# Gaurav14cs17/Bayer_Low_light_Image_Enhancement

Measured on AMD Instinct MI355X. Metric: megapixels/sec RawFormer-S 512x512 RAW->sRGB, higher is better.
Workload: dtype f32; 1 GPU; RawFormer-S(FLCA) dim=32, batch=8 of packed 4x512x512 synthetic Bayer per GPU; frames_per_gpu=8, variant=flca, weights=synthetic (seeded, random-init scale), parallelism=batch-sharded x1, device=AMD Radeon Graphics

## Files before the change

### bayer_low_light_image_enhancement_amd/csrc/rf_gemm1x1.hip

```cpp
#include <cstdio>
#include <cstdlib>
#include <type_traits>
#include "rf_common.h"

namespace rf {

__device__ __forceinline__ const float* kset_base(const Conv1x1Args& a, int b, int s) {
    const int k = 4 * s;
    const bool first = k < a.C1;
    const float* src = first ? a.x1 : a.x2;
    const size_t off = (size_t)b * (size_t)(first ? a.x1_bstride : a.x2_bstride) + (size_t)(first ? k : k - a.C1) * (size_t)a.P;
    return src + off;
}

__device__ __forceinline__ float4 ldv(const float* __restrict__ base, unsigned off) {
    return *reinterpret_cast<const float4*>(base + off);
}

template <int NCO>
__device__ __forceinline__ void zero_acc(f32x4 (&acc)[NCO][4]) {
#pragma unroll
    for (int t = 0; t < NCO; ++t)
#pragma unroll
        for (int g = 0; g < 4; ++g) acc[t][g] = (f32x4){0.f, 0.f, 0.f, 0.f};
}

template <class BP>
__device__ __forceinline__ void b3_split_pair(float xa, float xb, BP& bp, int g, int hp) {
    unsigned a0, a1, a2, b0, b1, b2;
    b3_split(xa, a0, a1, a2);
    b3_split(xb, b0, b1, b2);
    bp[g][0][hp] = b3_pack(a0, b0);
    bp[g][1][hp] = b3_pack(a1, b1);
    bp[g][2][hp] = b3_pack(a2, b2);
}

template <int NCO, bool RES>
__device__ __forceinline__ void epilogue(const Conv1x1Args& a, f32x4 (&acc)[NCO][4], int tfirst, int ntiles,
                                         const float* __restrict__ bias_l, const float4* res,
                                         int b, int p0, int kq, bool live) {
    const int P = a.P;
    float* outb = a.out + (size_t)b * a.out_bstride;
    if (a.mode == 0) {
        const unsigned voff = (unsigned)(4 * kq) * (unsigned)P + (unsigned)p0;
#pragma unroll
        for (int t = 0; t < NCO; ++t) {
            if (t >= ntiles) break;
#pragma unroll
            for (int r = 0; r < 4; ++r) {
                const int cu = 16 * (tfirst + t) + r;
                const float bs = bias_l[16 * t + 4 * kq + r];
                float v[4] = {acc[t][0][r] + bs, acc[t][1][r] + bs, acc[t][2][r] + bs, acc[t][3][r] + bs};
                if constexpr (RES) {
                    const float4 rv = res[t * 4 + r];
                    v[0] += rv.x; v[1] += rv.y; v[2] += rv.z; v[3] += rv.w;
                }
                if (a.act == 1 || a.act == 3) {
                    const float slope = a.act == 1 ? 0.2f : 0.1f;
#pragma unroll
                    for (int g = 0; g < 4; ++g) v[g] = v[g] > 0.f ? v[g] : slope * v[g];
                } else if (a.act == 2) {
#pragma unroll
                    for (int g = 0; g < 4; ++g) v[g] = fmaxf(v[g], 0.f);
                } else if (a.act == 4) {
#pragma unroll
                    for (int g = 0; g < 4; ++g) v[g] = fminf(fmaxf(v[g], 0.f), 1e4f);
                }
                if (live && cu + 4 * kq < a.Cout)
                    *reinterpret_cast<float4*>(outb + (size_t)cu * P + voff) = make_float4(v[0], v[1], v[2], v[3]);
            }
        }
    } else {
        const int w = a.w, w2 = 2 * a.w;
        const int ya = p0 / w, xa = p0 - ya * w;
        const int yb = (p0 + 2) / w, xb = (p0 + 2) - yb * w;
#pragma unroll
        for (int t = 0; t < NCO; ++t) {
            if (t >= ntiles) break;
            const int co = 16 * (tfirst + t) + 4 * kq;
            const int o = co >> 2;
            const float bs = bias_l[4 * t + kq];
            float* op = outb + (size_t)o * 4 * P;
            if (live && co < a.Cout) {
#pragma unroll
                for (int i = 0; i < 2; ++i) {
                    *reinterpret_cast<float4*>(op + (size_t)(2 * ya + i) * w2 + 2 * xa) =
                        make_float4(acc[t][0][2 * i] + bs, acc[t][0][2 * i + 1] + bs, acc[t][1][2 * i] + bs, acc[t][1][2 * i + 1] + bs);
                    *reinterpret_cast<float4*>(op + (size_t)(2 * yb + i) * w2 + 2 * xb) =
                        make_float4(acc[t][2][2 * i] + bs, acc[t][2][2 * i + 1] + bs, acc[t][3][2 * i] + bs, acc[t][3][2 * i + 1] + bs);
                }
            }
        }
    }
}

__device__ __forceinline__ void stage_bias(const Conv1x1Args& a, float* bias_l, int tbeg, int tpad, int tid) {
    if (a.mode == 0) {
        for (int i = tid; i < tpad * 16; i += 256) {
            const int co = 16 * tbeg + i;
            bias_l[i] = (a.bias && co < a.Cout) ? a.bias[co] : 0.f;
        }
    } else {
        for (int i = tid; i < tpad * 4; i += 256) {
            const int o = 4 * tbeg + i;
            bias_l[i] = (a.bias && 4 * o < a.Cout) ? a.bias[o] : 0.f;
        }
    }
}

template <int KS, bool LN, int RT, bool DBUF>
__global__ void __launch_bounds__(256, (KS <= 8 ? 3 : 2)) conv1x1_res_kernel(Conv1x1Args a, int ntw, int ngroups) {
    constexpr int NCO = 2;
    constexpr bool RES = RT > 0;
    extern __shared__ __attribute__((aligned(16))) float lds[];
    const int tid = threadIdx.x;
    const int lane = tid & 63, wave = tid >> 6;
    const int j = lane & 15, kq = lane >> 4;
    const int grp = blockIdx.x % ngroups;
    const int wg = blockIdx.x / ngroups, nwg = gridDim.x / ngroups;
    const int b = blockIdx.y;
    const int P = a.P;
    const int K = a.C1 + a.C2;
    const int NS = K >> 2;
    const int NT = (a.Cout + 15) >> 4;
    const int tbeg = grp * ntw;
    const int tcnt = (NT - tbeg < ntw) ? NT - tbeg : ntw;
    const int tpad = (tcnt + NCO - 1) / NCO * NCO;
    const int ntiles = (P + 255) >> 8;
    float* lds_w = lds;
    float* bias_l = lds + KS * tpad * 64;
    float* gam_l = bias_l + tpad * 16;
    float* bet_l = gam_l + 4 * KS;

    auto load_tile = [&](int tile, float4 (&dst)[KS]) {
        const int p0 = (tile * 4 + wave) * 64 + 4 * j;
        const unsigned voff = (unsigned)kq * (unsigned)P + (unsigned)(p0 < P ? p0 : 0);
#pragma unroll
        for (int s = 0; s < KS; ++s) dst[s] = ldv(kset_base(a, b, s < NS ? s : NS - 1), voff);
    };

    float4 xr[KS], xn[DBUF ? KS : 1];
    int tile = wg;
    load_tile(tile < ntiles ? tile : 0, xr);
    {
        const float* wp = a.wp + (size_t)b * a.wp_bstride;
        const int n4 = KS * tpad * 16;
        for (int idx = tid; idx < n4; idx += 256) {
            const int l4 = idx & 15;
            const int t = (idx >> 4) % tpad;
            const int s = (idx >> 4) / tpad;
            float4 v = make_float4(0.f, 0.f, 0.f, 0.f);
            if (t < tcnt && s < NS) v = *reinterpret_cast<const float4*>(wp + ((size_t)s * NT + tbeg + t) * 64 + l4 * 4);
            *reinterpret_cast<float4*>(lds_w + ((size_t)s * tpad + t) * 64 + l4 * 4) = v;
        }
        stage_bias(a, bias_l, tbeg, tpad, tid);
        if constexpr (LN) {
            for (int i = tid; i < 4 * KS; i += 256) {
                gam_l[i] = i < K ? a.ln_w[i] : 0.f;
                bet_l[i] = (a.ln_b && i < K) ? a.ln_b[i] : 0.f;
            }
        }
    }
    __syncthreads();

    for (; tile < ntiles; tile += nwg) {
        const int p0 = (tile * 4 + wave) * 64 + 4 * j;
        const bool live = p0 < P;
        const int tnext = tile + nwg;
        if constexpr (DBUF) {
            load_tile(tnext < ntiles ? tnext : tile, xn);
        }
        float4 res[RES ? RT * 4 : 1];
        if constexpr (RES) {
            const float* resb = a.res + (size_t)b * a.res_bstride;
            const unsigned voff = (unsigned)(4 * kq) * (unsigned)P + (unsigned)(live ? p0 : 0);
#pragma unroll
            for (int t = 0; t < RT; ++t)
#pragma unroll
                for (int r = 0; r < 4; ++r)
                    res[t * 4 + r] = ldv(resb + (size_t)(16 * (tbeg + (t < tcnt ? t : tcnt - 1)) + r) * P, voff);
        }
        if constexpr (LN) {
            float sum[4] = {0.f, 0.f, 0.f, 0.f};
#pragma unroll
            for (int s = 0; s < KS; ++s)
                if (s < NS) { sum[0] += xr[s].x; sum[1] += xr[s].y; sum[2] += xr[s].z; sum[3] += xr[s].w; }
            const float invK = 1.0f / (float)K;
            float mu[4], var[4] = {0.f, 0.f, 0.f, 0.f};
#pragma unroll
            for (int g = 0; g < 4; ++g) {
                sum[g] += __shfl_xor(sum[g], 16);
                sum[g] += __shfl_xor(sum[g], 32);
                mu[g] = sum[g] * invK;
            }
#pragma unroll
            for (int s = 0; s < KS; ++s) {
                if (s < NS) {
                    const float d0 = xr[s].x - mu[0], d1 = xr[s].y - mu[1], d2 = xr[s].z - mu[2], d3 = xr[s].w - mu[3];
                    var[0] = fmaf(d0, d0, var[0]); var[1] = fmaf(d1, d1, var[1]);
                    var[2] = fmaf(d2, d2, var[2]); var[3] = fmaf(d3, d3, var[3]);
                }
            }
            float rstd[4], sh[4];
#pragma unroll
            for (int g = 0; g < 4; ++g) {
                var[g] += __shfl_xor(var[g], 16);
                var[g] += __shfl_xor(var[g], 32);
                rstd[g] = 1.0f / sqrtf(var[g] * invK + a.ln_eps);
                sh[g] = a.ln_b ? mu[g] : 0.f;
            }
#pragma unroll
            for (int s = 0; s < KS; ++s) {
                const float gk = gam_l[4 * s + kq], bk = bet_l[4 * s + kq];
                xr[s].x = fmaf((xr[s].x - sh[0]) * rstd[0], gk, bk);
                xr[s].y = fmaf((xr[s].y - sh[1]) * rstd[1], gk, bk);
                xr[s].z = fmaf((xr[s].z - sh[2]) * rstd[2], gk, bk);
                xr[s].w = fmaf((xr[s].w - sh[3]) * rstd[3], gk, bk);
            }
        }
        auto do_group = [&](int tg, const float4* resp) {
            f32x4 acc[NCO][4];
            zero_acc(acc);
            const float* wl = lds_w + (size_t)tg * 64 + lane;
#pragma unroll
            for (int s = 0; s < KS; ++s) {
                const float xb[4] = {xr[s].x, xr[s].y, xr[s].z, xr[s].w};
#pragma unroll
                for (int t = 0; t < NCO; ++t) {
                    const float av = wl[((size_t)s * tpad + t) * 64];
#pragma unroll
                    for (int g = 0; g < 4; ++g)
                        acc[t][g] = __builtin_amdgcn_mfma_f32_16x16x4f32(av, xb[g], acc[t][g], 0, 0, 0);
                }
            }
            epilogue<NCO, RES>(a, acc, tbeg + tg, tcnt - tg, bias_l + (a.mode == 0 ? 16 : 4) * tg, resp, b, p0, kq, live);
        };
        if constexpr (RES) {
            do_group(0, &res[0]);
            if constexpr (RT > NCO) {
                if (tpad > NCO) do_group(NCO, &res[NCO * 4]);
            }
        } else {
#pragma unroll 1
            for (int tg = 0; tg < tpad; tg += NCO) do_group(tg, res);
        }
        if constexpr (DBUF) {
#pragma unroll
            for (int s = 0; s < KS; ++s) xr[s] = xn[s];
        } else {
            if (tnext < ntiles) load_tile(tnext, xr);
        }
    }
}

static constexpr int kStreamLnMaxK = 1024;

template <int NCO, int KCH, bool LN>
__global__ void __launch_bounds__(256, 2) conv1x1_stream_kernel(Conv1x1Args a, int ngroups) {
    __shared__ __attribute__((aligned(16))) float lds_w[2][KCH * NCO * 64];
    __shared__ float bias_l[NCO * 16];
    __shared__ float gam_l[LN ? kStreamLnMaxK : 4], bet_l[LN ? kStreamLnMaxK : 4];
    constexpr int WPT = KCH * NCO * 16 / 256;
    static_assert(KCH * NCO * 16 % 256 == 0, "weight chunk must split evenly over the workgroup");
    const int tid = threadIdx.x;
    const int lane = tid & 63, wave = tid >> 6;
    const int j = lane & 15, kq = lane >> 4;
    const int grp = blockIdx.x % ngroups;
    const int tile = blockIdx.x / ngroups;
    const int b = blockIdx.y;
    const int P = a.P;
    const int K = a.C1 + a.C2;
    const int NS = K >> 2;
    const int NT = (a.Cout + 15) >> 4;
    const int t0 = grp * NCO;
    const int tcnt = (NT - t0 < NCO) ? NT - t0 : NCO;
    const int nch = (NS + KCH - 1) / KCH;
    const int p0 = (tile * 4 + wave) * 64 + 4 * j;
    const bool live = p0 < P;
    const unsigned voff = (unsigned)kq * (unsigned)P + (unsigned)(live ? p0 : 0);
    const float* wp = a.wp + (size_t)b * a.wp_bstride;
    stage_bias(a, bias_l, t0, NCO, tid);
    if constexpr (LN) {
        for (int i = tid; i < 4 * nch * KCH; i += 256) {
            gam_l[i] = i < K ? a.ln_w[i] : 0.f;
            bet_l[i] = (a.ln_b && i < K) ? a.ln_b[i] : 0.f;
        }
    }

    f32x4 acc[NCO][4];
    zero_acc(acc);
    if (a.res && a.mode == 0) {
        const float* resb = a.res + (size_t)b * a.res_bstride;
        const unsigned vo = (unsigned)(live ? p0 : 0);
#pragma unroll
        for (int t = 0; t < NCO; ++t)
#pragma unroll
            for (int r = 0; r < 4; ++r) {
                const int co = 16 * (t0 + t) + 4 * kq + r;
                const bool ok = live && t < tcnt && co < a.Cout;
                const float4 rv = ldv(resb + (size_t)(ok ? co : 0) * P, vo);
                acc[t][0][r] = ok ? rv.x : 0.f; acc[t][1][r] = ok ? rv.y : 0.f;
                acc[t][2][r] = ok ? rv.z : 0.f; acc[t][3][r] = ok ? rv.w : 0.f;
            }
    }

    float lnA[4] = {1.f, 1.f, 1.f, 1.f}, lnB[4] = {0.f, 0.f, 0.f, 0.f};
    if constexpr (LN) {
        const float4 s4 = ldv(kset_base(a, b, 0), (unsigned)(live ? p0 : 0));
        const float sh[4] = {s4.x, s4.y, s4.z, s4.w};
        float s1[4] = {0.f, 0.f, 0.f, 0.f}, s2[4] = {0.f, 0.f, 0.f, 0.f};
#pragma unroll 16
        for (int s = 0; s < NS; ++s) {
            const float4 t = ldv(kset_base(a, b, s), voff);
            const float d[4] = {t.x - sh[0], t.y - sh[1], t.z - sh[2], t.w - sh[3]};
#pragma unroll
            for (int g = 0; g < 4; ++g) { s1[g] += d[g]; s2[g] = fmaf(d[g], d[g], s2[g]); }
        }
        const float invK = 1.0f / (float)K;
#pragma unroll
        for (int g = 0; g < 4; ++g) {
            s1[g] += __shfl_xor(s1[g], 16); s1[g] += __shfl_xor(s1[g], 32);
            s2[g] += __shfl_xor(s2[g], 16); s2[g] += __shfl_xor(s2[g], 32);
            const float md = s1[g] * invK;
            const float var = fmaxf(fmaf(-md, md, s2[g] * invK), 0.f);
            const float rstd = 1.0f / sqrtf(var + a.ln_eps);
            lnA[g] = rstd;
            lnB[g] = a.ln_b ? -(sh[g] + md) * rstd : 0.f;
        }
    }

    float4 xa[KCH], xb_[KCH], wr[WPT];
    auto load_x_chunk = [&](int c, float4 (&dst)[KCH]) {
#pragma unroll
        for (int i = 0; i < KCH; ++i) {
            const int s = c * KCH + i;
            dst[i] = ldv(kset_base(a, b, s < NS ? s : NS - 1), voff);
        }
    };
    auto load_w_chunk = [&](int c) {
#pragma unroll
        for (int i = 0; i < WPT; ++i) {
            const int idx = tid + 256 * i;
            const int l4 = idx & 15, t = (idx >> 4) % NCO, s = c * KCH + (idx >> 4) / NCO;
            const bool ok = s < NS && t < tcnt;
            const float4 v = *reinterpret_cast<const float4*>(wp + ((size_t)(ok ? s : 0) * NT + t0 + (ok ? t : 0)) * 64 + l4 * 4);
            wr[i] = ok ? v : make_float4(0.f, 0.f, 0.f, 0.f);
        }
    };
    auto store_w_chunk = [&](int buf) {
#pragma unroll
        for (int i = 0; i < WPT; ++i) *reinterpret_cast<float4*>(&lds_w[buf][(tid + 256 * i) * 4]) = wr[i];
    };
    auto chunk = [&](int c, float4 (&xc)[KCH], float4 (&xn)[KCH]) {
        if (c + 1 < nch) {
            load_x_chunk(c + 1, xn);
            load_w_chunk(c + 1);
        }
        const float* wl = &lds_w[c & 1][lane];
#pragma unroll
        for (int i = 0; i < KCH; ++i) {
            float xv[4] = {xc[i].x, xc[i].y, xc[i].z, xc[i].w};
            if constexpr (LN) {
                const int k = 4 * (c * KCH + i) + kq;
                const float gk = gam_l[k], bk = bet_l[k];
#pragma unroll
                for (int g = 0; g < 4; ++g) xv[g] = fmaf(fmaf(xv[g], lnA[g], lnB[g]), gk, bk);
            }
#pragma unroll
            for (int t = 0; t < NCO; ++t) {
                const float av = wl[(i * NCO + t) * 64];
#pragma unroll
                for (int g = 0; g < 4; ++g)
                    acc[t][g] = __builtin_amdgcn_mfma_f32_16x16x4f32(av, xv[g], acc[t][g], 0, 0, 0);
            }
        }
        if (c + 1 < nch) store_w_chunk((c + 1) & 1);
        __syncthreads();
    };

    load_x_chunk(0, xa);
    load_w_chunk(0);
    store_w_chunk(0);
    __syncthreads();
    for (int c = 0; c < nch; c += 2) {
        chunk(c, xa, xb_);
        if (c + 1 < nch) chunk(c + 1, xb_, xa);
    }
    epilogue<NCO, false>(a, acc, t0, tcnt, bias_l, nullptr, b, p0, kq, live);
}


__device__ __forceinline__ void b3_load_x_block(float4 (&xr)[8], const float* xb1, const float* xb2, const float* xb3, int C1, int C2, int C3,
                                                int c, int kq, unsigned P, unsigned pl) {
    const int cb = 32 * c;
    const bool first = cb < C1, third = cb >= C1 + C2;
    const float* src = first ? xb1 : third ? xb3 : xb2;
    const int cloc = first ? cb : third ? cb - C1 - C2 : cb - C1, cmax = (first ? C1 : third ? C3 : C2) - 1;
#pragma unroll
    for (int i = 0; i < 8; ++i) {
        int ch = cloc + 8 * kq + i;
        ch = ch < cmax ? ch : cmax;
        xr[i] = ldv(src, (unsigned)ch * P + pl);
    }
}

template <int NCO, bool LN, bool PAIR = false>
__global__ void __launch_bounds__(PAIR ? 512 : 256, 2) conv1x1_b3_kernel(Conv1x1Args a, int ngroups) {
    static_assert(!(PAIR && LN), "the paired form has no LayerNorm prologue");
    constexpr int NH = PAIR ? 2 : 1;
    __shared__ __attribute__((aligned(16))) u32x4 lds_w[NH * 2][NCO * 3 * 64];
    __shared__ float bias_l[NH * NCO * 16];
    __shared__ float gam_l[LN ? kStreamLnMaxK : 4], bet_l[LN ? kStreamLnMaxK : 4];
    constexpr int WPT = (NCO * 3 * 64 + 255) / 256;
    const int tid = PAIR ? threadIdx.x & 255 : threadIdx.x;
    const int half = PAIR ? threadIdx.x >> 8 : 0;
    const int lane = tid & 63, wave = tid >> 6;
    const int j = lane & 15, kq = lane >> 4;
    unsigned unit = 0, gp = 0, utiles = 1;
    if constexpr (PAIR) {
        utiles = (unsigned)(a.P + 255) >> 8;
        if (!conv1x1_group_map(blockIdx.x, (unsigned)a.B * utiles, (unsigned)(ngroups + 1) >> 1, &unit, &gp)) return;
    }
    const int grp = PAIR ? 2 * (int)gp + half : blockIdx.x % ngroups;
    const int tile = PAIR ? unit % utiles : blockIdx.x / ngroups;
    const int b = PAIR ? unit / utiles : blockIdx.y;
    const int P = a.P;
    const int K = a.C1 + a.C2 + a.C3;
    const int NB = (K + 31) >> 5;
    const int NT = (a.Cout + 15) >> 4;
    const bool idle = PAIR && grp >= ngroups;
    const int t0 = idle ? 0 : grp * NCO;
    const int tcnt = idle ? 0 : (NT - t0 < NCO) ? NT - t0 : NCO;
    const int p0 = (tile * 4 + wave) * 64 + 4 * j;
    const bool live = p0 < P;
    const unsigned pl = (unsigned)(live ? p0 : 0);
    const u32x4* wp3 = reinterpret_cast<const u32x4*>(reinterpret_cast<const float*>(a.wp3) + (size_t)b * a.wp3_bstride);
    stage_bias(a, bias_l + half * NCO * 16, t0, NCO, tid);
    if constexpr (LN) {
        for (int i = tid; i < 32 * NB; i += 256) {
            gam_l[i] = i < K ? a.ln_w[i] : 0.f;
            bet_l[i] = (a.ln_b && i < K) ? a.ln_b[i] : 0.f;
        }
    }

    f32x4 acc[NCO][4];
#pragma unroll
    for (int t = 0; t < NCO; ++t)
#pragma unroll
        for (int g = 0; g < 4; ++g) acc[t][g] = (f32x4){0.f, 0.f, 0.f, 0.f};
    if (a.res && a.mode == 0) {
        const float* resb = a.res + (size_t)b * a.res_bstride;
#pragma unroll
        for (int t = 0; t < NCO; ++t)
#pragma unroll
            for (int r = 0; r < 4; ++r) {
                const int co = 16 * (t0 + t) + 4 * kq + r;
                const bool ok = live && t < tcnt && co < a.Cout;
                const float4 rv = ldv(resb + (size_t)(ok ? co : 0) * P, pl);
                acc[t][0][r] = ok ? rv.x : 0.f; acc[t][1][r] = ok ? rv.y : 0.f;
                acc[t][2][r] = ok ? rv.z : 0.f; acc[t][3][r] = ok ? rv.w : 0.f;
            }
    }

    float lnA[4] = {1.f, 1.f, 1.f, 1.f}, lnB[4] = {0.f, 0.f, 0.f, 0.f};
    if constexpr (LN) {
        const unsigned voff = (unsigned)kq * (unsigned)P + pl;
        const float4 s4 = ldv(kset_base(a, b, 0), pl);
        const float sh[4] = {s4.x, s4.y, s4.z, s4.w};
        float s1[4] = {0.f, 0.f, 0.f, 0.f}, s2[4] = {0.f, 0.f, 0.f, 0.f};
#pragma unroll 16
        for (int s = 0; s < (K >> 2); ++s) {
            const float4 t = ldv(kset_base(a, b, s), voff);
            const float d[4] = {t.x - sh[0], t.y - sh[1], t.z - sh[2], t.w - sh[3]};
#pragma unroll
            for (int g = 0; g < 4; ++g) { s1[g] += d[g]; s2[g] = fmaf(d[g], d[g], s2[g]); }
        }
        const float invK = 1.0f / (float)K;
#pragma unroll
        for (int g = 0; g < 4; ++g) {
            s1[g] += __shfl_xor(s1[g], 16); s1[g] += __shfl_xor(s1[g], 32);
            s2[g] += __shfl_xor(s2[g], 16); s2[g] += __shfl_xor(s2[g], 32);
            const float md = s1[g] * invK;
            const float var = fmaxf(fmaf(-md, md, s2[g] * invK), 0.f);
            const float rstd = 1.0f / sqrtf(var + a.ln_eps);
            lnA[g] = rstd;
            lnB[g] = a.ln_b ? -(sh[g] + md) * rstd : 0.f;
        }
    }

    float4 xr[8];
    u32x4 wr[WPT];
    const float* const xb1 = a.x1 + (size_t)b * (size_t)a.x1_bstride;
    const float* const xb2 = a.x2 + (size_t)b * (size_t)a.x2_bstride;
    const float* const xb3 = a.x3 + (size_t)b * (size_t)a.x3_bstride;
    auto load_x_block = [&](int c) { b3_load_x_block(xr, xb1, xb2, xb3, a.C1, a.C2, a.C3, c, kq, (unsigned)P, pl); };
    auto load_w_block = [&](int c) {
#pragma unroll
        for (int i = 0; i < WPT; ++i) {
            const int idx = tid + 256 * i;
            const int t = idx / 192, rem = idx - t * 192;
            const bool ok = idx < NCO * 192 && t < tcnt;
            const u32x4 v = wp3[((size_t)c * NT + t0 + (ok ? t : 0)) * 192 + (ok ? rem : 0)];
            wr[i] = ok ? v : (u32x4){0u, 0u, 0u, 0u};
        }
    };
    auto store_w_block = [&](int buf) {
#pragma unroll
        for (int i = 0; i < WPT; ++i)
            if (tid + 256 * i < NCO * 192) lds_w[2 * half + buf][tid + 256 * i] = wr[i];
    };

    load_x_block(0);
    load_w_block(0);
    store_w_block(0);
    __syncthreads();
    for (int c = 0; c < NB; ++c) {
        u32x4 bp[4][3];
#pragma unroll
        for (int hp = 0; hp < 4; ++hp) {
            float xa[4] = {xr[2 * hp].x, xr[2 * hp].y, xr[2 * hp].z, xr[2 * hp].w};
            float xb[4] = {xr[2 * hp + 1].x, xr[2 * hp + 1].y, xr[2 * hp + 1].z, xr[2 * hp + 1].w};
            if constexpr (LN) {
                const int k = 32 * c + 8 * kq + 2 * hp;
                const float ga = gam_l[k], ba = bet_l[k], gb = gam_l[k + 1], bb = bet_l[k + 1];
#pragma unroll
                for (int g = 0; g < 4; ++g) {
                    xa[g] = fmaf(fmaf(xa[g], lnA[g], lnB[g]), ga, ba);
                    xb[g] = fmaf(fmaf(xb[g], lnA[g], lnB[g]), gb, bb);
                }
            }
#pragma unroll
            for (int g = 0; g < 4; ++g) b3_split_pair(xa[g], xb[g], bp, g, hp);
        }
        if (c + 1 < NB) {
            load_x_block(c + 1);
            load_w_block(c + 1);
        }
        const u32x4* wl = &lds_w[2 * half + (c & 1)][lane];
#pragma unroll
        for (int t = 0; t < NCO; ++t) {
            const u32x4 ap[3] = {wl[(t * 3 + 0) * 64], wl[(t * 3 + 1) * 64], wl[(t * 3 + 2) * 64]};
            b3_mfma4(ap, bp, acc[t]);
        }
        if (c + 1 < NB) store_w_block((c + 1) & 1);
        __syncthreads();
    }
    epilogue<NCO, false>(a, acc, t0, tcnt, bias_l + half * NCO * 16, nullptr, b, p0, kq, live);
}

template <int KB, int NCO, bool RESIDENT>
__device__ __forceinline__ void b3_ln_tiles(const Conv1x1Args& a, const int tpw, u32x4* __restrict__ Bl, float* __restrict__ red,
                                            const float* __restrict__ bias_l) {
    constexpr int KPW = KB >= 4 ? KB / 4 : 1;
    constexpr int CPT = KB >= 4 ? 8 : 4;
    constexpr int K = 32 * KB;
    constexpr int STEPS = KB * NCO, RING = RESIDENT ? STEPS : KB > 4 ? 12 : (STEPS < 5 ? STEPS : 5);
    constexpr int AHEAD = RESIDENT ? STEPS : RING - 1;
    constexpr int XSTEP = (KB == 4 && NCO == 3) ? STEPS - NCO : STEPS - RING;
    const int tid = threadIdx.x, lane = tid & 63, wave = __builtin_amdgcn_readfirstlane(tid >> 6);
    const int j = lane & 15, kq = lane >> 4;
    const int b = blockIdx.y, P = a.P;
    const int NT = a.Cout >> 4;
    const int ntile = (P + 63) >> 6;
    const int tw0 = ((int)blockIdx.z * 4 + wave) * tpw;
    const float* xb = a.x1 + (size_t)b * a.x1_bstride;
    float* outb = a.out + (size_t)b * a.out_bstride;
    const char* wp3 = reinterpret_cast<const char*>(reinterpret_cast<const float*>(a.wp3) + (size_t)b * a.wp3_bstride);
    const unsigned aoff = 16u * (unsigned)lane;

    const int kb0 = KB >= 4 ? wave * KPW : wave >> 1;
    const int cwave = KB >= 4 ? 0 : 4 * (wave & 1);
    const int cbase = 8 * kq + cwave;
    float4 xr[KPW][CPT];
    auto load_x = [&](int tile, bool exists) {
        const int q0 = tile * 64 + 4 * j;
        size_t xoff = exists ? (size_t)(8 * kq) * (size_t)P + (size_t)(q0 < P ? q0 : tile * 64) : (size_t)0;
        asm volatile("" : "+v"(xoff));
#pragma unroll
        for (int i = 0; i < KPW; ++i)
#pragma unroll
            for (int c = 0; c < CPT; ++c) xr[i][c] = *reinterpret_cast<const float4*>(xb + (size_t)(32 * (kb0 + i) + cwave + c) * (size_t)P + xoff);
    };
    u32x4 A[RING][3];
    auto load_a = [&](int slot, int step, int t0) {
        const int kb = step / NCO, t = step - kb * NCO;
#pragma unroll
        for (int pc = 0; pc < 3; ++pc)
            A[slot][pc] = *reinterpret_cast<const u32x4*>(wp3 + (((size_t)kb * NT + t0 + t) * 192 + pc * 64) * 16 + aoff);
    };
    load_x(blockIdx.x, true);
#pragma unroll
    for (int i = 0; i < AHEAD; ++i) load_a(i, i, tw0);
    constexpr bool LNREG = KB != 4;
    float gam[LNREG ? KPW : 1][CPT], bet[LNREG ? KPW : 1][CPT];
    if constexpr (LNREG) {
#pragma unroll
        for (int i = 0; i < KPW; ++i)
#pragma unroll
            for (int c = 0; c < CPT; ++c) {
                const int k = 32 * (kb0 + i) + cbase + c;
                gam[i][c] = a.ln_w[k];
                bet[i][c] = a.ln_b ? a.ln_b[k] : 0.f;
            }
    }
    __builtin_amdgcn_s_waitcnt(0x0F70);

    for (int tile = blockIdx.x; tile < ntile; tile += gridDim.x) {
    const int tnext = tile + (int)gridDim.x;
    const bool more = tnext < ntile;
    const int q0 = tile * 64 + 4 * j;
    const int p0 = q0 < P ? q0 : tile * 64;
    float mean[4], rstd[4];
    {
        float s[4] = {0.f, 0.f, 0.f, 0.f};
#pragma unroll
        for (int i = 0; i < KPW; ++i)
#pragma unroll
            for (int c = 0; c < CPT; ++c) { s[0] += xr[i][c].x; s[1] += xr[i][c].y; s[2] += xr[i][c].z; s[3] += xr[i][c].w; }
#pragma unroll
        for (int g = 0; g < 4; ++g) { s[g] += __shfl_xor(s[g], 16); s[g] += __shfl_xor(s[g], 32); }
        if (kq == 0) *reinterpret_cast<float4*>(red + wave * 64 + 4 * j) = make_float4(s[0], s[1], s[2], s[3]);
        __syncthreads();
        const float4 r0 = *reinterpret_cast<const float4*>(red + 4 * j), r1 = *reinterpret_cast<const float4*>(red + 64 + 4 * j);
        const float4 r2 = *reinterpret_cast<const float4*>(red + 128 + 4 * j), r3 = *reinterpret_cast<const float4*>(red + 192 + 4 * j);
        mean[0] = (((r0.x + r1.x) + r2.x) + r3.x) * (1.0f / K); mean[1] = (((r0.y + r1.y) + r2.y) + r3.y) * (1.0f / K);
        mean[2] = (((r0.z + r1.z) + r2.z) + r3.z) * (1.0f / K); mean[3] = (((r0.w + r1.w) + r2.w) + r3.w) * (1.0f / K);
        float v[4] = {0.f, 0.f, 0.f, 0.f};
#pragma unroll
        for (int i = 0; i < KPW; ++i)
#pragma unroll
            for (int c = 0; c < CPT; ++c) {
                const float d0 = xr[i][c].x - mean[0], d1 = xr[i][c].y - mean[1], d2 = xr[i][c].z - mean[2], d3 = xr[i][c].w - mean[3];
                v[0] = fmaf(d0, d0, v[0]); v[1] = fmaf(d1, d1, v[1]); v[2] = fmaf(d2, d2, v[2]); v[3] = fmaf(d3, d3, v[3]);
            }
#pragma unroll
        for (int g = 0; g < 4; ++g) { v[g] += __shfl_xor(v[g], 16); v[g] += __shfl_xor(v[g], 32); }
        if (kq == 0) *reinterpret_cast<float4*>(red + 256 + wave * 64 + 4 * j) = make_float4(v[0], v[1], v[2], v[3]);
        __syncthreads();
        const float4 q0 = *reinterpret_cast<const float4*>(red + 256 + 4 * j), q1 = *reinterpret_cast<const float4*>(red + 320 + 4 * j);
        const float4 q2 = *reinterpret_cast<const float4*>(red + 384 + 4 * j), q3 = *reinterpret_cast<const float4*>(red + 448 + 4 * j);
        rstd[0] = 1.0f / sqrtf((((q0.x + q1.x) + q2.x) + q3.x) * (1.0f / K) + a.ln_eps);
        rstd[1] = 1.0f / sqrtf((((q0.y + q1.y) + q2.y) + q3.y) * (1.0f / K) + a.ln_eps);
        rstd[2] = 1.0f / sqrtf((((q0.z + q1.z) + q2.z) + q3.z) * (1.0f / K) + a.ln_eps);
        rstd[3] = 1.0f / sqrtf((((q0.w + q1.w) + q2.w) + q3.w) * (1.0f / K) + a.ln_eps);
    }
#pragma unroll
    for (int i = 0; i < KPW; ++i) {
        const int kb = kb0 + i;
        unsigned bpd[4][3][CPT / 2];
#pragma unroll
        for (int hp = 0; hp < CPT / 2; ++hp) {
            const int k = 32 * kb + cbase + 2 * hp;
            const float ga = LNREG ? gam[LNREG ? i : 0][2 * hp] : a.ln_w[k], gb = LNREG ? gam[LNREG ? i : 0][2 * hp + 1] : a.ln_w[k + 1];
            const float ba = LNREG ? bet[LNREG ? i : 0][2 * hp] : a.ln_b ? a.ln_b[k] : 0.f, bb = LNREG ? bet[LNREG ? i : 0][2 * hp + 1] : a.ln_b ? a.ln_b[k + 1] : 0.f;
            const float xa[4] = {xr[i][2 * hp].x, xr[i][2 * hp].y, xr[i][2 * hp].z, xr[i][2 * hp].w};
            const float xc[4] = {xr[i][2 * hp + 1].x, xr[i][2 * hp + 1].y, xr[i][2 * hp + 1].z, xr[i][2 * hp + 1].w};
#pragma unroll
            for (int g = 0; g < 4; ++g) {
                const float mu = a.ln_b ? mean[g] : 0.f;
                b3_split_pair(fmaf((xa[g] - mu) * rstd[g], ga, ba), fmaf((xc[g] - mu) * rstd[g], gb, bb), bpd, g, hp);
            }
        }
#pragma unroll
        for (int g = 0; g < 4; ++g)
#pragma unroll
            for (int pc = 0; pc < 3; ++pc) {
                u32x4* dst = &Bl[((kb * 4 + g) * 3 + pc) * 64 + lane];
                if constexpr (CPT == 8) *dst = (u32x4){bpd[g][pc][0], bpd[g][pc][1], bpd[g][pc][2], bpd[g][pc][3]};
                else reinterpret_cast<uint2*>(dst)[wave & 1] = make_uint2(bpd[g][pc][0], bpd[g][pc][1]);
            }
    }
    __syncthreads();
    if constexpr (RESIDENT) load_x(tnext, more);
    unsigned soff = 4u * ((unsigned)(4 * kq) * (unsigned)P + (unsigned)p0);
    asm volatile("" : "+v"(soff));

    auto run_chunk = [&](const int t0, auto last_chunk) {
        constexpr bool LAST = decltype(last_chunk)::value;
        f32x4 acc[NCO][4];
#pragma unroll
        for (int t = 0; t < NCO; ++t)
#pragma unroll
            for (int g = 0; g < 4; ++g) acc[t][g] = (f32x4){0.f, 0.f, 0.f, 0.f};
        u32x4 bp[2][4][3];
        auto load_b = [&](int buf, int kb, int first, int last) {
#pragma unroll
            for (int i = first; i < last; ++i) bp[buf][i / 3][i % 3] = Bl[(kb * 12 + i) * 64 + lane];
        };
        load_b(0, 0, 0, 12);
#pragma unroll
        for (int step = 0; step < STEPS; ++step) {
            const int kb = step / NCO, t = step % NCO;
            if constexpr (!RESIDENT) {
                if (step + RING - 1 < STEPS) load_a((step + RING - 1) % RING, step + RING - 1, t0);
                if (LAST && step == XSTEP) {
                    __builtin_amdgcn_sched_barrier(0);
                    load_x(tnext, more);
                }
            }
            if (kb + 1 < KB) load_b((kb + 1) & 1, kb + 1, 12 * t / NCO, 12 * (t + 1) / NCO);
            b3_mfma4(A[step % RING], bp[kb & 1], acc[t]);
            __builtin_amdgcn_sched_barrier(0);
        }
        if constexpr (!RESIDENT) {
#pragma unroll
            for (int i = 0; i < RING - 1; ++i) load_a(i, i, LAST ? tw0 : t0 + NCO);
            __builtin_amdgcn_sched_barrier(0);
        }
#pragma unroll
        for (int t = 0; t < NCO; ++t)
#pragma unroll
            for (int r = 0; r < 4; ++r) {
                const float bs = bias_l[16 * (t0 + t) + 4 * kq + r];
                float v[4] = {acc[t][0][r] + bs, acc[t][1][r] + bs, acc[t][2][r] + bs, acc[t][3][r] + bs};
                if (a.act == 1 || a.act == 3) {
                    const float slope = a.act == 1 ? 0.2f : 0.1f;
#pragma unroll
                    for (int g = 0; g < 4; ++g) v[g] = v[g] > 0.f ? v[g] : slope * v[g];
                } else if (a.act == 2) {
#pragma unroll
                    for (int g = 0; g < 4; ++g) v[g] = fmaxf(v[g], 0.f);
                } else if (a.act == 4) {
#pragma unroll
                    for (int g = 0; g < 4; ++g) v[g] = fminf(fmaxf(v[g], 0.f), 1e4f);
                }
                *reinterpret_cast<float4*>(reinterpret_cast<char*>(outb + (size_t)(16 * (t0 + t) + r) * (size_t)P) + soff) = make_float4(v[0], v[1], v[2], v[3]);
            }
    };
    if constexpr (!RESIDENT)
        for (int t0 = tw0; t0 + NCO < tw0 + tpw; t0 += NCO) run_chunk(t0, std::false_type{});
    run_chunk(tw0 + tpw - NCO, std::true_type{});
    }
}

template <int KB, int NCO>
__global__ void __launch_bounds__(256, KB <= 4 ? 2 : 1) conv1x1_b3_ln_kernel(Conv1x1Args a, int tpw) {
    __shared__ __attribute__((aligned(16))) u32x4 Bl[KB * 768];
    __shared__ __attribute__((aligned(16))) float red[2 * 4 * 64];
    __shared__ float bias_l[1024];
    for (int i = threadIdx.x; i < a.Cout; i += 256) bias_l[i] = a.bias ? a.bias[i] : 0.f;
    if constexpr (KB == 2) {
        if (tpw == NCO) return b3_ln_tiles<KB, NCO, true>(a, tpw, Bl, red, bias_l);
    }
    b3_ln_tiles<KB, NCO, false>(a, tpw, Bl, red, bias_l);
}

__global__ void __launch_bounds__(256) conv1x1_scalar_kernel(Conv1x1Args a) {
    const int P = a.P, K = a.C1 + a.C2, NT = (a.Cout + 15) >> 4;
    const int b = blockIdx.y;
    const float* wp = a.wp + (size_t)b * a.wp_bstride;
    for (int p = blockIdx.x * 256 + threadIdx.x; p < P; p += gridDim.x * 256) {
        auto xat = [&](int k) {
            return (k < a.C1) ? a.x1[(size_t)b * a.x1_bstride + (size_t)k * P + p]
                              : a.x2[(size_t)b * a.x2_bstride + (size_t)(k - a.C1) * P + p];
        };
        float mu = 0.f, rstd = 1.f;
        if (a.ln_w) {
            for (int k = 0; k < K; ++k) mu += xat(k);
            mu /= (float)K;
            float var = 0.f;
            for (int k = 0; k < K; ++k) { const float d = xat(k) - mu; var = fmaf(d, d, var); }
            rstd = 1.0f / sqrtf(var / (float)K + a.ln_eps);
            if (!a.ln_b) mu = 0.f;
        }
        for (int co = 0; co < a.Cout; ++co) {
            float s = 0.f;
            for (int k = 0; k < K; ++k) {
                float xv = xat(k);
                if (a.ln_w) xv = fmaf((xv - mu) * rstd, a.ln_w[k], a.ln_b ? a.ln_b[k] : 0.f);
                s = fmaf(wp[((size_t)(k >> 2) * NT + (co >> 4)) * 64 + (co & 15) + 16 * (k & 3)], xv, s);
            }
            if (a.mode == 0) {
                s += a.bias ? a.bias[co] : 0.f;
                if (a.res) s += a.res[(size_t)b * a.res_bstride + (size_t)co * P + p];
                if (a.act == 1) s = s > 0.f ? s : 0.2f * s;
                else if (a.act == 2) s = fmaxf(s, 0.f);
                else if (a.act == 3) s = s > 0.f ? s : 0.1f * s;
                else if (a.act == 4) s = fminf(fmaxf(s, 0.f), 1e4f);
                a.out[(size_t)b * a.out_bstride + (size_t)co * P + p] = s;
            } else {
                const int o = co >> 2, y = p / a.w, x = p - y * a.w;
                s += a.bias ? a.bias[o] : 0.f;
                a.out[(size_t)b * a.out_bstride + (size_t)o * 4 * P + (size_t)(2 * y + ((co >> 1) & 1)) * (2 * a.w) + 2 * x + (co & 1)] = s;
            }
        }
    }
}

enum { kScalar, kRes, kStream, kB3, kB3Ln };
struct Conv1x1Inst {
    const char* key;
    int family, targ[4];
    unsigned block;
    void (*launch)(const Conv1x1Args&, const Conv1x1Plan&, hipStream_t);
};
#define RF_GRID dim3(p.grid[0], p.grid[1], p.grid[2]), p.block, p.lds, st
#define RF_INST(FAMILY, BLOCK, KERNEL, KARGS, ...)                                      \
    {#KERNEL "<" #__VA_ARGS__ ">", FAMILY, {__VA_ARGS__}, BLOCK,                        \
     [](const Conv1x1Args& a, const Conv1x1Plan& p, hipStream_t st) { KERNEL<__VA_ARGS__><<<RF_GRID>>> KARGS; }}
#define RF_RES(...) RF_INST(kRes, 256, conv1x1_res_kernel, (a, p.karg[0], p.karg[1]), __VA_ARGS__)
#define RF_RES6(KS, DBUF4)              \
    RF_RES(KS, true, 4, DBUF4), RF_RES(KS, false, 4, DBUF4), RF_RES(KS, true, 2, true), RF_RES(KS, false, 2, true), RF_RES(KS, true, 0, true), RF_RES(KS, false, 0, true)
#define RF_STREAM(...) RF_INST(kStream, 256, conv1x1_stream_kernel, (a, p.karg[0]), __VA_ARGS__)
#define RF_B3(BLOCK, ...) RF_INST(kB3, BLOCK, conv1x1_b3_kernel, (a, p.karg[0]), __VA_ARGS__)
#define RF_B3LN(...) RF_INST(kB3Ln, 256, conv1x1_b3_ln_kernel, (a, p.karg[0]), __VA_ARGS__)
static const Conv1x1Inst kInst[] = {
    {"conv1x1_scalar_kernel", kScalar, {}, 256, [](const Conv1x1Args& a, const Conv1x1Plan& p, hipStream_t st) { conv1x1_scalar_kernel<<<RF_GRID>>>(a); }},
    RF_B3LN(2, 3), RF_B3LN(2, 2), RF_B3LN(4, 3), RF_B3LN(4, 2), RF_B3LN(8, 4), RF_B3LN(8, 3), RF_B3LN(8, 2),
    RF_B3(512, 6, false, true), RF_B3(512, 4, false, true), RF_B3(256, 6, false), RF_B3(256, 2, false), RF_B3(256, 4, true), RF_B3(256, 4, false),
    RF_RES6(4, true), RF_RES6(8, true), RF_RES6(12, false), RF_RES6(16, false),
    RF_RES(24, false, 0, false), RF_RES(32, false, 0, false),
    RF_STREAM(8, 4, true), RF_STREAM(8, 4, false), RF_STREAM(4, 8, true), RF_STREAM(4, 8, false),
};
#undef RF_GRID

static int find_inst(int family, int t0, int t1, int t2, Conv1x1Plan* p) {
    const int want[3] = {t0, t1, t2};
    for (const Conv1x1Inst& r : kInst) {
        bool ok = r.family == family;
        for (int k = 0; k < 3; ++k) ok = ok && (want[k] < 0 || want[k] == r.targ[k]);
        if (ok) { p->inst = (int)(&r - kInst); p->key = r.key; p->block = r.block; return RF_OK; }
    }
    RF_CHECK_ARG(false, "conv1x1: no kernel instantiation for family %d <%d, %d, %d>", family, t0, t1, t2);
}

static bool b3_ln_supported(const Conv1x1Args& a, int* nco) {
    const int K = a.C1 + a.C2;
    if (!(a.ln_w && a.wp3 && a.C2 == 0 && (K == 64 || K == 128 || K == 256) && a.mode == 0 && !a.res && a.Cout % 64 == 0 && a.Cout <= 1024 &&
          aligned16(a.wp3) && a.wp3_bstride % 4 == 0))
        return false;
    const int tpw = a.Cout / 64;
    *nco = (K == 256 && tpw % 4 == 0) ? 4 : tpw % 3 == 0 ? 3 : tpw % 2 == 0 ? 2 : 0;
    return *nco != 0;
}

static bool b3_supported(const Conv1x1Args& a) {
    const int K = a.C1 + a.C2 + a.C3;
    return K >= 128 && a.C1 % 8 == 0 && a.C2 % 8 == 0 && a.C3 % 8 == 0 && (a.C2 + a.C3 == 0 || a.C1 % 32 == 0) &&
           (a.C3 == 0 || a.C2 % 32 == 0) && (!a.ln_w || (K <= kStreamLnMaxK && a.C3 == 0)) && aligned16(a.wp3) && (a.wp3_bstride % 4 == 0);
}

int plan_conv1x1(const Conv1x1Args& a, Conv1x1Plan* p) {
    bool b3_ok = a.wp3 != nullptr;
    int force_pair = -1;
#ifdef RF_DIAG
    if (getenv("RF_NO_B3")) b3_ok = false;
    if (const char* e = getenv("RF_B3_PAIR")) force_pair = e[0] != '0';
#endif
    RF_CHECK_ARG(a.B > 0 && a.P > 0 && a.C1 > 0 && a.C2 >= 0 && a.Cout > 0, "conv1x1: bad sizes B=%d P=%d C1=%d C2=%d Cout=%d",
                 a.B, a.P, a.C1, a.C2, a.Cout);
    RF_CHECK_ARG(a.C1 % 4 == 0 && a.C2 % 4 == 0, "conv1x1: input channel counts (%d, %d) must be multiples of 4", a.C1, a.C2);
    RF_CHECK_ARG(a.C2 == 0 || a.x2 != nullptr, "conv1x1: second source missing");
    RF_CHECK_ARG(a.C3 >= 0 && a.C3 % 4 == 0 && (a.C3 == 0 || (a.x3 != nullptr && a.C2 > 0)), "conv1x1: bad third source (C3 = %d)", a.C3);
    RF_CHECK_ARG(a.mode == 0 || (a.Cout % 4 == 0 && a.w > 0 && a.P % a.w == 0 && !a.res), "conv1x1: bad ConvTranspose geometry");
    RF_CHECK_ARG(a.B <= 65535 && (double)a.P * 4.0 * 16.0 < 4.0e9, "conv1x1: batch %d / plane %d too large", a.B, a.P);
    const int K = a.C1 + a.C2 + a.C3;
    const int NS = K / 4, NT = cdiv(a.Cout, 16);
    const int ptiles = cdiv(a.P, 256);
    const long units = (long)ptiles * a.B;
    bool vec = (a.P % 4 == 0) && aligned16(a.x1) && aligned16(a.out) && (a.x1_bstride % 4 == 0) && (a.out_bstride % 4 == 0);
    if (a.x2) vec = vec && aligned16(a.x2) && (a.x2_bstride % 4 == 0);
    if (a.C3) vec = vec && aligned16(a.x3) && (a.x3_bstride % 4 == 0);
    if (a.res) vec = vec && aligned16(a.res) && (a.res_bstride % 4 == 0);
    if (a.mode == 1) vec = vec && (a.w % 2 == 0);
    const bool ln = a.ln_w != nullptr;
    const double px = (double)a.B * a.P;
    *p = Conv1x1Plan{};
    p->flops = 2.0 * K * a.Cout * px;
    p->bytes = 4.0 * px * (K + a.Cout + (a.res ? a.Cout : 0));
    p->grid[1] = (unsigned)a.B; p->grid[2] = 1;
    int nco_ln = 0;
    const bool ln_once = b3_ln_supported(a, &nco_ln);
    p->ln_single_pass = !ln || a.C1 + a.C2 <= 64 || ln_once;
    const bool use_b3 = b3_ok && b3_supported(a);
    RF_CHECK_ARG(a.C3 == 0 || (use_b3 && vec && !a.ln_w && !(a.res && a.Cout % 16 != 0)), "conv1x1: three sources need the bf16x3 kernel (K = %d, P = %d)", K, a.P);
    if (!vec || (a.res && a.Cout % 16 != 0) || (ln && K > kStreamLnMaxK)) {
        p->grid[0] = (unsigned)(cdiv(a.P, 256) < 4096 ? cdiv(a.P, 256) : 4096);
        return find_inst(kScalar, -1, -1, -1, p);
    }
    if (b3_ok && ln_once) {
        const int kb = K / 32;
        int tpw = a.Cout / 64;
        const int slots = (kb <= 4 ? 2 : 1) * 256;
        int gx = slots / a.B;
        gx = gx < 1 ? 1 : gx;
        gx = gx < cdiv(a.P, 64) ? gx : cdiv(a.P, 64);
        int zs = 1;
        if ((long)gx * a.B < 128)
            for (int z = tpw / nco_ln; z > 1; --z)
                if ((tpw / nco_ln) % z == 0 && (long)gx * a.B * z <= 512) { zs = z; break; }
        p->grid[0] = (unsigned)gx; p->grid[2] = (unsigned)zs;
        p->karg[0] = tpw / zs;
        return find_inst(kB3Ln, kb, nco_ln, -1, p);
    }
    if (use_b3) {
        int nco = (!ln && (NT % 6 == 0 || (NT % 4 != 0 && NT > 8))) ? 6 : 4;
        const bool pair = !ln && cdiv(NT, nco) > 1 && (force_pair >= 0 ? force_pair != 0 : units * cdiv(cdiv(NT, nco), 2) >= 256);
        if (!pair && !ln && nco == 4 && NT % 2 == 0 && units * cdiv(NT, 4) < 256) nco = 2;
        const int ngroups = cdiv(NT, nco);
        const long pair_ids = (units + 7) / 8 * 8 * cdiv(ngroups, 2);
        RF_CHECK_ARG(!pair || pair_ids < (1L << 31), "conv1x1: %ld pixel tiles x %d output groups is too large a grid", units, ngroups);
        p->karg[0] = ngroups;
        if (pair) { p->grid[0] = conv1x1_group_grid((unsigned)units, (unsigned)cdiv(ngroups, 2)); p->grid[1] = 1; }
        else p->grid[0] = (unsigned)(ptiles * ngroups);
        return find_inst(kB3, nco, ln, pair, p);
    }
    if (NS <= 16 || (NS <= 32 && !ln && !a.res)) {
        const int ks = NS <= 4 ? 4 : NS <= 8 ? 8 : NS <= 12 ? 12 : NS <= 16 ? 16 : NS <= 24 ? 24 : 32;
        int cap = (240 / ks) & ~1;
        if (a.res && cap > 4) cap = 4;
        if (a.res && (ks <= 8 || ln) && cap > 2) cap = 2;
        const int ntw = NT < cap ? NT : cap;
        const int ngroups = cdiv(NT, ntw);
        const int tpad = cdiv(ntw, 2) * 2;
        p->lds = ((size_t)ks * tpad * 64 + tpad * 16 + 8 * ks) * sizeof(float);
        const int slots = 256 * (ks <= 8 ? 3 : 2);
        int wgs = cdiv(slots, a.B * ngroups);
        if (wgs > ptiles) wgs = ptiles;
        p->grid[0] = (unsigned)(wgs * ngroups);
        p->karg[0] = ntw; p->karg[1] = ngroups;
        return find_inst(kRes, ks, ln, a.res ? (ntw > 2 ? 4 : 2) : 0, p);
    }
    int nco = (NT % 8 == 0 || NT > 12) ? 8 : 4;
    if (nco == 8) {
        const long cost8 = ((units * cdiv(NT, 8) + 511) / 512) * 8, cost4 = ((units * cdiv(NT, 4) + 511) / 512) * 4;
        if (cost4 < cost8) nco = 4;
    }
    p->karg[0] = cdiv(NT, nco);
    p->grid[0] = (unsigned)(ptiles * p->karg[0]);
    return find_inst(kStream, nco, -1, ln, p);
}

bool conv1x1_ln_single_pass(const Conv1x1Args& a) {
    Conv1x1Plan p;
    return plan_conv1x1(a, &p) != RF_OK || p.ln_single_pass;
}

int launch_conv1x1(const Conv1x1Args& a, hipStream_t st) {
    Conv1x1Plan p;
    RF_TRY(plan_conv1x1(a, &p));
    {
        ProfScope prof(st, p.key, p.flops, p.bytes);
        kInst[p.inst].launch(a, p, st);
    }
    return check_launch("conv1x1");
}

}
```

Measured before the change: 1118 MP/s.

## Prefetch weight blocks two stages ahead and peel the 1x1 GEMM loop

```diff
diff --git a/bayer_low_light_image_enhancement_amd/csrc/rf_gemm1x1.hip b/bayer_low_light_image_enhancement_amd/csrc/rf_gemm1x1.hip
--- a/bayer_low_light_image_enhancement_amd/csrc/rf_gemm1x1.hip
+++ b/bayer_low_light_image_enhancement_amd/csrc/rf_gemm1x1.hip
@@ -448,20 +448,6 @@
     for (int t = 0; t < NCO; ++t)
 #pragma unroll
         for (int g = 0; g < 4; ++g) acc[t][g] = (f32x4){0.f, 0.f, 0.f, 0.f};
-    if (a.res && a.mode == 0) {
-        const float* resb = a.res + (size_t)b * a.res_bstride;
-#pragma unroll
-        for (int t = 0; t < NCO; ++t)
-#pragma unroll
-            for (int r = 0; r < 4; ++r) {
-                const int co = 16 * (t0 + t) + 4 * kq + r;
-                const bool ok = live && t < tcnt && co < a.Cout;
-                const float4 rv = ldv(resb + (size_t)(ok ? co : 0) * P, pl);
-                acc[t][0][r] = ok ? rv.x : 0.f; acc[t][1][r] = ok ? rv.y : 0.f;
-                acc[t][2][r] = ok ? rv.z : 0.f; acc[t][3][r] = ok ? rv.w : 0.f;
-            }
-    }
-
     float lnA[4] = {1.f, 1.f, 1.f, 1.f}, lnB[4] = {0.f, 0.f, 0.f, 0.f};
     if constexpr (LN) {
         const unsigned voff = (unsigned)kq * (unsigned)P + pl;
@@ -493,33 +479,34 @@
     const float* const xb1 = a.x1 + (size_t)b * (size_t)a.x1_bstride;
     const float* const xb2 = a.x2 + (size_t)b * (size_t)a.x2_bstride;
     const float* const xb3 = a.x3 + (size_t)b * (size_t)a.x3_bstride;
-    auto load_x_block = [&](int c) { b3_load_x_block(xr, xb1, xb2, xb3, a.C1, a.C2, a.C3, c, kq, (unsigned)P, pl); };
-    auto load_w_block = [&](int c) {
+    auto load_x_block = [&](int c, float4 (&xs)[8]) { b3_load_x_block(xs, xb1, xb2, xb3, a.C1, a.C2, a.C3, c, kq, (unsigned)P, pl); };
+    unsigned woff[WPT], wmask[WPT];
+#pragma unroll
+    for (int i = 0; i < WPT; ++i) {
+        const int idx = tid + 256 * i;
+        const int t = idx / 192, rem = idx - t * 192;
+        const bool ok = idx < NCO * 192 && t < tcnt;
+        wmask[i] = ok ? 0xffffffffu : 0u;
+        woff[i] = (unsigned)((t0 + (ok ? t : 0)) * 192 + (ok ? rem : 0));
+    }
+    auto load_w_block = [&](int c, u32x4 (&w)[WPT]) {
+        const u32x4* wc = wp3 + (size_t)c * NT * 192;
 #pragma unroll
         for (int i = 0; i < WPT; ++i) {
-            const int idx = tid + 256 * i;
-            const int t = idx / 192, rem = idx - t * 192;
-            const bool ok = idx < NCO * 192 && t < tcnt;
-            const u32x4 v = wp3[((size_t)c * NT + t0 + (ok ? t : 0)) * 192 + (ok ? rem : 0)];
-            wr[i] = ok ? v : (u32x4){0u, 0u, 0u, 0u};
-        }
-    };
-    auto store_w_block = [&](int buf) {
+            w[i] = wc[woff[i]];
+        }
+    };
+    auto store_w_block = [&](int buf, const u32x4 (&w)[WPT]) {
 #pragma unroll
         for (int i = 0; i < WPT; ++i)
-            if (tid + 256 * i < NCO * 192) lds_w[2 * half + buf][tid + 256 * i] = wr[i];
-    };
-
-    load_x_block(0);
-    load_w_block(0);
-    store_w_block(0);
-    __syncthreads();
-    for (int c = 0; c < NB; ++c) {
+            if (tid + 256 * i < NCO * 192) lds_w[2 * half + buf][tid + 256 * i] = w[i] & wmask[i];
+    };
+    auto block = [&](int c, float4 (&xs)[8], auto LX, auto LW, auto SW) {
         u32x4 bp[4][3];
 #pragma unroll
         for (int hp = 0; hp < 4; ++hp) {
-            float xa[4] = {xr[2 * hp].x, xr[2 * hp].y, xr[2 * hp].z, xr[2 * hp].w};
-            float xb[4] = {xr[2 * hp + 1].x, xr[2 * hp + 1].y, xr[2 * hp + 1].z, xr[2 * hp + 1].w};
+            float xa[4] = {xs[2 * hp].x, xs[2 * hp].y, xs[2 * hp].z, xs[2 * hp].w};
+            float xb[4] = {xs[2 * hp + 1].x, xs[2 * hp + 1].y, xs[2 * hp + 1].z, xs[2 * hp + 1].w};
             if constexpr (LN) {
                 const int k = 32 * c + 8 * kq + 2 * hp;
                 const float ga = gam_l[k], ba = bet_l[k], gb = gam_l[k + 1], bb = bet_l[k + 1];
@@ -532,9 +519,9 @@
 #pragma unroll
             for (int g = 0; g < 4; ++g) b3_split_pair(xa[g], xb[g], bp, g, hp);
         }
-        if (c + 1 < NB) {
-            load_x_block(c + 1);
-            load_w_block(c + 1);
+        if constexpr (decltype(LX)::value) {
+            load_x_block(c + 1, xs);
+            __builtin_amdgcn_sched_barrier(0);
         }
         const u32x4* wl = &lds_w[2 * half + (c & 1)][lane];
 #pragma unroll
@@ -542,9 +529,38 @@
             const u32x4 ap[3] = {wl[(t * 3 + 0) * 64], wl[(t * 3 + 1) * 64], wl[(t * 3 + 2) * 64]};
             b3_mfma4(ap, bp, acc[t]);
         }
-        if (c + 1 < NB) store_w_block((c + 1) & 1);
+        __builtin_amdgcn_sched_barrier(0);
+        if constexpr (decltype(SW)::value) store_w_block((c + 1) & 1, wr);
+        if constexpr (decltype(LW)::value) load_w_block(c + 2, wr);
+        if constexpr (decltype(SW)::value) __syncthreads();
+    };
+    constexpr std::true_type yes{};
+    constexpr std::false_type no{};
+
+    {
+        u32x4 w0[WPT];
+        load_w_block(0, w0);
+        load_x_block(0, xr);
+        load_w_block(1, wr);
+        if (a.res && a.mode == 0) {
+            const float* resb = a.res + (size_t)b * a.res_bstride;
+#pragma unroll
+            for (int t = 0; t < NCO; ++t)
+#pragma unroll
+                for (int r = 0; r < 4; ++r) {
+                    const int co = 16 * (t0 + t) + 4 * kq + r;
+                    const bool ok = live && t < tcnt && co < a.Cout;
+                    const float4 rv = ldv(resb + (size_t)(ok ? co : 0) * P, pl);
+                    acc[t][0][r] = ok ? rv.x : 0.f; acc[t][1][r] = ok ? rv.y : 0.f;
+                    acc[t][2][r] = ok ? rv.z : 0.f; acc[t][3][r] = ok ? rv.w : 0.f;
+                }
+        }
+        store_w_block(0, w0);
         __syncthreads();
     }
+    for (int c = 0; c < NB - 2; ++c) block(c, xr, yes, yes, yes);
+    block(NB - 2, xr, yes, no, yes);
+    block(NB - 1, xr, no, no, no);
     epilogue<NCO, false>(a, acc, t0, tcnt, bias_l + half * NCO * 16, nullptr, b, p0, kq, live);
 }
 
```

Measured after the change: 1124 MP/s (median of 6 runs). About the same (+0.6%).
